# mhvk/baseband

Measured on AMD Instinct MI355X. Metric: decoded Msamples/s, VDIF 2-bit 1-thread (scan + index + decode, input resident in HBM), higher is better.
Workload: dtype float32; 1 GPU; cfg2: synthetic 8.000 GiB per GPU single-thread VDIF, 2-bit real, 1 channel, EDV 0, 8032-byte frames; input_memory=arena, output_memory=torch.empty, 127.5 GiB (above the readers' 64 GiB arena block limit)

## Files before the change

baseband_amd/_lib.py:

```python
import ctypes as C
import os

import torch

_HERE = os.path.dirname(os.path.abspath(__file__))
EXPERIMENTS = os.environ.get('BB_EXPERIMENTS', '') not in ('', '0')
LIB_PATH = os.path.join(_HERE, 'libbbdecode_exp.so' if EXPERIMENTS else 'libbbdecode.so')

BB_OK = 0
BB_EIO = -5
BB_EINVAL = -22
BB_ERANGE = -34
BB_ENOTSUP = -95

CODER_VDIF = 0
CODER_MARK5B = 1
CODER_INT = 2

OUT_F32 = 0
OUT_F16 = 1
OUT_BF16 = 2

FRAME_OK = 0x1
FRAME_INVALID = 0x2
# ... 3 lines not shown
TUNE_ENCODE_DIRECT = 5
TUNE_GATHER_BYTES = 6
TUNE_TILES_PER_WAVE = 7
TUNE_TILED_STAGE = 10
TUNE_MKBF_CHANNELS = 11
TUNE_GATHER_CHUNKS = 12
TUNE_SEG_TILES = 13
TUNE_WORK_STRIPES = 18
TUNE_XPOSE = 19
TUNE_XPOSE_ROWS = 20
TUNE_M4_WIDEN = 22
TUNE_SELECT_BYTES = 23
TUNE_LUT_TILES = 24
TUNE_M4_TILES = 26
TUNE_XPOSE_TC = 27
TUNE_XPOSE_MIN_NC = 28
TUNE_ENCODE_RUNS = 30
TUNE_GATHER_GLDS = 36
TUNE_ENCODE_STRIPES = 38
TUNE_SELECT_PICK = 39
TUNE_PICK_BYTES = 40
TUNE_VDIF8_LDS_GIB = 41
TUNE_TOUCH_MIB = 42
TUNE_FLAT_VARIANT = 0
TUNE_NT_STORES = 1
TUNE_NT_LOADS = 3
TUNE_TILES_PER_WAVE_8BIT = 8
TUNE_LDS_PAD = 9
TUNE_FRONT_GROUP = 14
TUNE_FRONT_STEPS = 15
TUNE_OUT_STRIPE_W = 16
TUNE_OUT_STRIPE_S = 17
TUNE_BYTE_LUT = 21
TUNE_LUT_SMALL = 25
TUNE_FLAT8_LDS = 29
TUNE_BURST = 31
TUNE_COPY = 35
TUNE_M4_LDS = 37
TUNE_BURST_BYTES = 32
TUNE_BURST_PERIOD = 33
TUNE_BURST_WAVES = 34


class BBError(RuntimeError):
    def __init__(self, code, where):
        self.code = code
# ... 162 lines not shown
    ('bb_count_states_bins', C.c_int, [_vp, _sz, _vp, _sz, C.POINTER(StatesParams), C.c_uint64, C.c_uint64,
                                       C.c_uint64, _vp, _sz, _vp]),
    ('bb_count_states_bins_check', C.c_int, [C.POINTER(StatesParams), C.c_uint64]),
    ('bb_i8_moments', C.c_int, [_vp, _sz, _vp, _sz, C.POINTER(MomentsParams), _vp, _sz, _vp]),
    ('bb_i8_moments_check', C.c_int, [C.POINTER(MomentsParams)]),
    ('bb_i8_coherence', C.c_int, [_vp, _sz, _vp, _sz, C.POINTER(MomentsParams), _vp, _sz, _vp]),
    ('bb_i8_coherence_check', C.c_int, [C.POINTER(MomentsParams)]),
    ('bb_repack_frames', C.c_int, [_vp, _sz, _vp, _sz, C.POINTER(RepackParams), _vp, _sz, _vp]),
    ('bb_repack_check', C.c_int, [C.POINTER(RepackParams)]),
    ('bb_requant_frames', C.c_int, [_vp, _sz, _vp, _sz, C.POINTER(RequantParams), _vp, _sz, _vp]),
    ('bb_requant_check', C.c_int, [C.POINTER(RequantParams)]),
    ('bb_recode_frames', C.c_int, [_vp, _sz, _vp, _sz, C.POINTER(RecodeParams), _vp, _sz, _vp]),
    ('bb_recode_check', C.c_int, [C.POINTER(RecodeParams)]),
    ('bb_recode_frames_tables', C.c_int, [_vp, _sz, _vp, _sz, C.POINTER(RecodeParams), _vp, _sz, _vp, _sz, _vp]),
    ('bb_recode_tables_check', C.c_int, [C.POINTER(RecodeParams)]),
    ('bb_fetch_counter', C.c_int, [_vp, _vp, _vp, _vp]),
    ('bb_mark5b_read_window', C.c_int, [_vp, _sz, C.POINTER(Mark5BScanParams), _sz, _sz, C.POINTER(DecodeParams),
                                        _vp, C.c_int, _vp, _vp, _vp, _sz, _sz, _vp, _vp, _vp, _vp]),
    ('bb_mark4_read_window', C.c_int, [_vp, _sz, C.POINTER(Mark4ScanParams), _sz, _sz,
                                       C.POINTER(Mark4DecodeParams), C.c_int, _vp, _vp, _vp, _sz, _sz, _vp, _vp,
                                       _vp, _vp]),
    ('bb_vdif_read_window', C.c_int, [_vp, _sz, C.POINTER(VDIFScanParams), _sz, _vp, _sz, C.POINTER(DecodeParams),
                                      _vp, C.c_int, _vp, _vp, _vp, _sz, C.c_uint32, _sz, _vp, _vp, _vp, _vp]),
    ('bb_mark4_scan', C.c_int, [_vp, _sz, C.POINTER(Mark4ScanParams), _vp, _sz, _vp]),
    ('bb_mark4_locate', C.c_int, [_vp, _sz, C.c_int, _vp, _sz, _vp, _vp]),
    ('bb_mark4_header_crc', C.c_int, [_vp, _sz, C.c_int, _vp, C.c_int64, _sz, _vp, _vp]),
    ('bb_mark4_scan_at', C.c_int, [_vp, _sz, C.POINTER(Mark4ScanParams), _vp, _sz, _vp, _vp]),
    ('bb_decode_mark4', C.c_int, [_vp, _sz, _vp, _sz, C.POINTER(Mark4DecodeParams), _vp, _sz, _vp]),
    ('bb_decode_mark4_select', C.c_int, [_vp, _sz, _vp, _sz, C.POINTER(Mark4DecodeParams), C.c_int,
                                         _vp, _sz, _vp]),
    ('bb_decode_i8_tiled', C.c_int, [_vp, _sz, _vp, _sz, C.POINTER(TiledParams), _vp, _sz, _vp]),
    ('bb_encode_flat', C.c_int, [_vp, _sz, C.c_int, C.c_int, _vp, _sz, _vp]),
    ('bb_encode_mark4', C.c_int, [_vp, _sz, C.c_int, C.POINTER(C.c_uint8), C.POINTER(C.c_uint8), _vp, _sz, _vp]),
    ('bb_tune', C.c_int, [C.c_int, C.c_int]),
    ('bb_arena_create', C.c_int, [_sz, C.POINTER(_vp)]),
    ('bb_arena_alloc', C.c_int, [_vp, _sz, C.POINTER(_vp)]),
    ('bb_arena_prepare', C.c_int, [_vp, _sz]),
    ('bb_arena_owns', C.c_int, [_vp, _vp]),
    ('bb_arena_free', C.c_int, [_vp, _vp]),
    ('bb_arena_trim', C.c_int, [_vp, C.POINTER(_sz)]),
    ('bb_arena_get_stats', C.c_int, [_vp, C.POINTER(ArenaStats)]),
    ('bb_arena_destroy', C.c_int, [_vp]),
]

EXPERIMENT_SIGNATURES = [
    ('bb_debug_trace', C.c_int, [_vp]),
# ... 157 lines not shown
```

baseband_amd/base/base.py:

```python
import operator
import io
import os
import threading
import warnings

import numpy as np
import torch

from .. import _lib
from .. import kernels
from ..placement import empty_output
from .. import placement as _placement
from ..staging import host_image, WindowPipeline
from .packed import PackedBytesMixin
from .quantities import as_time, as_timedelta, is_time_like, is_duration_like

_SIDE_SCAN = os.environ.get('BB_SIDE_SCAN', '1') not in ('0', 'no', 'off')
_scan_streams = {}
_scan_streams_lock = threading.Lock()

__all__ = ['FileBase', 'VLBIFileReaderBase', 'GPUStreamReaderBase',
           'HeaderNotFoundError']


# ... 389 lines not shown
        sub = 'subset={0}, '.format(self.subset) if getattr(self, 'subset', None) else ''
        return ("<{cls} name={name} offset={offset}\n"
                "    sample_rate={rate}, samples_per_frame={spf},\n"
                "    sample_shape={shape}, bps={bps},\n"
                "    {sub}start_time={start}>"
                .format(cls=type(self).__name__, name=getattr(self.fh_raw, 'name', None), offset=attr('offset'),
                        rate=attr('sample_rate'), spf=attr('samples_per_frame'), shape=attr('sample_shape'),
                        bps=attr('bps'), sub=sub, start=attr('start_time')))

    def seekable(self):
        return True

    @property
    def info(self):
        from .info import StreamReaderInfo
        cached = self.__dict__.get('_info')
        if cached is None or cached.verify != self.verify or cached.closed != self.closed:
            cached = self.__dict__['_info'] = StreamReaderInfo(self)
        return cached

    def close(self):
        self._closed = True
        self._drop_windows()
        self._staged = self._sink = None
        self._have = []
        if self._pipeline is not None:
            self._pipeline.release()
            self._pipeline = None
        self.fh_raw.close()
        self._unregister()

    def __enter__(self):
        return self

    def __exit__(self, *exc):
        self.close()

    _within_np = None
    _within_dev = None

    @property
    def _within(self):
        if self._within_np is None:
            return None
        if self._within_dev is None:
            kernels.require_gpu()
# ... 436 lines not shown
                        device=dev, priority=int(os.environ.get('BB_SIDE_SCAN_PRIORITY', '-1')))
            self._scan_stream = st
        key = (resident.data_ptr(), resident.numel(), None if self._nbad is None else self._nbad.data_ptr(),
               self._side_state_key())
        if self._scan_ready_for != key:
            ev = torch.cuda.Event()
            ev.record(torch.cuda.current_stream(dev))
            self._scan_stream.wait_event(ev)
            self._scan_ready_for = key
        return self._scan_stream

    def _side_state_key(self):
        return None

    def _zero_nbad(self):
        if self._nbad is not None:
            if self._scan_stream is not None:
                self._scan_stream.synchronize()
            self._nbad.zero_()
            if self._scan_stream is not None:
                torch.cuda.current_stream(self._nbad.device).synchronize()

    def _reset_checks(self):
        self._nmissing, self._checked, self._check_recs = 0, False, 0
        self._zero_nbad()

    def _fill_request(self, out, count):
        spf = self.samples_per_frame
        first, off0 = divmod(self.offset, spf)
        stop = self.offset + count
        last = -(-stop // spf) if count else first
        flat = self._direct_target(out)
        body0, body1 = first + (1 if off0 else 0), stop // spf
        if flat is not None and count and body1 > body0:
            row = flat.numel() // count
            o0 = body0 * spf - self.offset
            self._read_sets(body0, body1, flat[o0 * row:(o0 + (body1 - body0) * spf) * row])
            if off0:
                head = self._squeeze_and_subset(self._read_sets_as(first, body0, flat.dtype))
                out[:o0] = head[off0:]
            if body1 < last:
                ntail = stop - body1 * spf
                tail = self._squeeze_and_subset(self._read_sets_as(body1, last, flat.dtype))
                out[count - ntail:] = tail[:ntail]
            return out, True
        data = self._read_sets(first, last) if out is None else self._read_sets_as(first, last, self._out_elem(out))
        return data[off0:off0 + count], False
# ... 39 lines not shown
        return flat.reshape(data.shape)

    def _decode_sets(self, first, last, into, elem):
        kernels.require_gpu()
        self._last_scan_side = None
        nsets = last - first
        spf = self.samples_per_frame
        ncomp = 2 if self.complex_data else 1
        row = int(np.prod(self._decode_shape)) * ncomp
        flat = into if into is not None else kernels.empty_decoded(nsets * spf * row, dtype=elem)
        set_nbytes = self._set_nbytes
        resident = self._resident_bytes() if nsets else None
        if resident is None and nsets and self._have:
            lo_ = self._file_offset0 + first * set_nbytes
            hi_ = min(self._file_offset0 + (last + (1 if self.verify else 0)) * set_nbytes,
                      len(self._image()))
            if self._has_bytes(min(lo_, hi_), hi_):
                resident = self._sink[:len(self._image())]
        if resident is not None:
            lo = min(self._file_offset0 + first * set_nbytes, resident.numel())
            look = 1 if self.verify else 0
            hi = max(lo, min(self._file_offset0 + (last + look) * set_nbytes, resident.numel()))
            win = self._device_window(resident, lo, hi)
            if (self.verify and _SIDE_SCAN and nsets * set_nbytes >= (16 << 20)
                    and win.data_ptr() == resident.data_ptr() + lo):
                self._prepare_window_state(win.device)
                self._scan_side = self._scan_stream_for(resident)
            try:
                self._process_window(win, first, last, flat)
            except Exception:
                self._reset_checks()
                raise
            finally:
                self._last_scan_side, self._scan_side = self._scan_side, None
        elif nsets and nsets * set_nbytes * 8 <= self.window_bytes:
            self._read_small(first, last, flat, spf * row)
        elif nsets:
            image = self._image()
            per_win = max(1, self.pipeline_window_bytes // set_nbytes)
            if self._pipeline is None:
                self._pipeline = WindowPipeline(image, (per_win + 1) * set_nbytes)
            sink = self._sink_tensor()
            ranges, spans = [], []
            starts, s = [], first
            for size in ((max(1, per_win // 16), max(1, per_win // 4)) if self.ramp_windows else ()):
                if s < last:
                    starts.append(s)
                    s += size
            starts.extend(range(s, last, per_win))
            for i, s in enumerate(starts):
                e = min(last, starts[i + 1] if i + 1 < len(starts) else s + per_win)
                lo = min(self._file_offset0 + s * set_nbytes, len(image))
                look = 1 if (self.verify and e == last) else 0
                hi = max(lo, min(self._file_offset0 + (e + look) * set_nbytes, len(image)))
                ranges.append((lo, hi))
                spans.append((s, e))

            def process(dbuf, i):
                s, e = spans[i]
                o = flat[(s - first) * spf * row:(e - first) * spf * row]
                self._process_window(self._device_window(dbuf, 0, dbuf.numel()), s, e, o)

            try:
                self._pipeline.run(ranges, process, sink=sink)
            except Exception:
                self._reset_checks()
                raise
            if sink is not None:
                for lo, hi in ranges:
                    self._mark_have(lo, hi)
        if self.complex_data:
            flat = torch.view_as_complex(flat.view(-1, 2))
        return flat.reshape((nsets * spf,) + tuple(self._decode_shape))

    _ahead = None
    _ahead_bytes0 = 256 << 10
    _ahead_bytes = 256 << 10

    def _read_small(self, first, last, flat, set_floats):
        from ..staging import upload
        set_nbytes = self._set_nbytes
        image = self._image()
        total = (len(image) - self._file_offset0) // set_nbytes
        look = 1 if self.verify else 0
        need_end = min(last + look, total)
        ahead = self._ahead
        if ahead is None or first < ahead[0] or need_end > ahead[1]:
            if ahead is not None and ahead[0] <= first <= ahead[1]:
                self._ahead_bytes = min(self.window_bytes, 4 * self._ahead_bytes)
            else:
                self._ahead_bytes = self._ahead_bytes0
            per_win = max(last - first + look, self._ahead_bytes // set_nbytes)
            end = min(total, first + per_win)
            lo = self._file_offset0 + first * set_nbytes
            hi = max(lo, self._file_offset0 + end * set_nbytes)
            dev = upload(image[lo:hi])
# ... 13 lines not shown
    def _note_checked(self, nrecs, missing=0):
        self._check_recs += int(nrecs)
        self._nmissing += int(missing)
        self._checked = True

    def _verdict_targets(self):
        if self._nbad is None:
            self._nbad = torch.zeros(1, dtype=torch.int32, device='cuda')
        if self._check_event is None:
            self._check_event = torch.cuda.Event()
            self._check_event.record()
        return self._nbad, self._check_event.cuda_event

    _check_recs = 0
    _check_event = None
    _check_stream = None
    _nbad_host = None

    def _resolve_checks(self, quiet=False):
        checked, self._checked = self._checked, False
        if not self.verify or not checked:
            return True
        nrecs, self._check_recs = self._check_recs, 0
        if nrecs < 2048:
            nbad = int(self._nbad.item()) + self._nmissing
        else:
            if self._check_stream is None:
                self._check_stream = torch.cuda.Stream(device=self._nbad.device)
                self._nbad_host = torch.zeros(1, dtype=torch.int32, pin_memory=True)
            on_scan = self._last_scan_side
            kernels.fetch_counter(self._nbad, self._nbad_host, None if on_scan is not None else self._check_event,
                                  on_scan if on_scan is not None else self._check_stream)
            nbad = int(self._nbad_host[0]) + self._nmissing
        self._nmissing = 0
        if nbad:
            self._zero_nbad()
            if quiet:
                return False
            msg = ("problem loading frame: {} frame header(s) failed verification "
                   "(bad sync/invariants or unexpected time index)".format(nbad))
            if self.verify == 'fix':
                if self._can_relocate and not self._relocated:
                    return False
                warnings.warn(msg + "; affected samples were set to fill_value.")
            else:
                err = self._verification_error(msg)
                if err is None and self._can_relocate:
                    return False
                raise err if err is not None else ValueError("wrong frame number. " + msg)
        return True

    def _verification_error(self, msg):
        return ValueError("wrong frame number. " + msg)

    _asked = None

# ... 125 lines not shown
```

baseband_amd/csrc/bbdecode.hip:

```cpp
#include "bb_common.h"
#include "k_scan.h"
#include "k_flat.h"
#if BB_EXP
#include "k_exp.h"
#endif
#include "k_lut.h"
#include "k_lds.h"
#include "k_half.h"
#include "bb_half_host.h"
#include "k_copy.h"
#include "k_states.h"
#include "k_state_bins.h"
#include "k_repack.h"
#include "k_requant.h"
#include "k_recode.h"
#include "k_recode_tables.h"
#include "k_moments.h"
#include "k_coherence.h"
#include "k_tfpick.h"
#if BB_EXP
#include "k_burst.h"
#endif
#include "k_gather.h"
#include "k_pick.h"
// ... 141 lines not shown
#define BB_LOCATE_GRID 65536ull

struct bb_knob {
    int v;
    int load() const { return v; }
    bb_knob &operator=(int x) { v = x; return *this; }
};
thread_local bb_knob g_tune_blocks{0};
thread_local bb_knob g_tune_tile_elems{8192};
thread_local bb_knob g_tune_encode_direct{0};
thread_local bb_knob g_tune_gather_bytes{8192};
thread_local bb_knob g_tune_tiled_stage{1};
thread_local bb_knob g_tune_seg_tiles{0};
thread_local bb_knob g_tune_gather_chunks{32};
thread_local bb_knob g_tune_mkbf_tc{32};
thread_local bb_knob g_tune_rows_tiles{8};
thread_local bb_knob g_tune_lut_tpw{0};
static int touch_mib_default()
{
    static const int v = [] { const char *e = getenv("BB_TOUCH_MIB"); char *end = nullptr; const long x = e && *e ? strtol(e, &end, 10) : 256; return (e && *e && end == e) || x < 0 || x > (1 << 20) ? 256 : (int)x; }();
    return v;
}
thread_local bb_knob g_tune_touch_mib{touch_mib_default()};
thread_local bb_knob g_tune_vdif8_lds_gib{20};
thread_local bb_knob g_tune_select_pick{1};
thread_local bb_knob g_tune_pick_bytes{4096};
thread_local bb_knob g_tune_select_bytes{16384};
thread_local bb_knob g_tune_m4_tiles{BB_M4_TPW};
thread_local bb_knob g_tune_m4_widen{1};
thread_local bb_knob g_tune_xpose_rows{0};
#if BB_EXP
thread_local bb_knob g_tune_flat8_lds{0};
#endif
thread_local bb_knob g_tune_encode_runs{0};
thread_local bb_knob g_tune_encode_lw{0};
thread_local bb_knob g_tune_xpose_tc{0};
thread_local bb_knob g_tune_xpose_min_nc{8};
thread_local bb_knob g_tune_xpose{1};
thread_local bb_knob g_tune_gather_glds{-1};
thread_local bb_knob g_tune_order_lw{-1};
#if BB_EXP
thread_local bb_knob g_tune_m4_lds{0};
thread_local bb_knob g_tune_copy{0};
thread_local bb_knob g_tune_variant{5};
thread_local bb_knob g_tune_burst{0};
thread_local bb_knob g_tune_burst_bytes{65536};
// ... 451 lines not shown
    switch (knob) {
        case BB_TUNE_BLOCKS:       g_tune_blocks = value;  return BB_OK;
        case BB_TUNE_TILE_ELEMS:   g_tune_tile_elems = value > 0 ? value : 8192; return BB_OK;
        case BB_TUNE_ENCODE_DIRECT: g_tune_encode_direct = value; return BB_OK;
        case BB_TUNE_TILES_PER_WAVE:
            g_tune_rows_tiles = (value >= 1 && value <= 8) ? value : 8;
#if BB_EXP
            g_tune_tpw = (value >= 1 && value <= 16) ? value : 12;
#endif
            return BB_OK;
        case BB_TUNE_GATHER_BYTES: g_tune_gather_bytes = value > 0 ? value : 8192; return BB_OK;
        case BB_TUNE_TILED_STAGE: g_tune_tiled_stage = value; return BB_OK;
        case BB_TUNE_SEG_TILES: g_tune_seg_tiles = (value >= 1 && value <= 4096) ? value : 0; return BB_OK;
        case BB_TUNE_GATHER_CHUNKS: g_tune_gather_chunks = value > 0 ? value : 32; return BB_OK;
        case BB_TUNE_MKBF_CHANNELS: g_tune_mkbf_tc = (value >= 2 && value <= 64 && !(value & 1)) ? value : 32; return BB_OK;
        case BB_TUNE_M4_WIDEN: g_tune_m4_widen = value; return BB_OK;
        case BB_TUNE_M4_TILES: g_tune_m4_tiles = (value >= 1 && value <= BB_M4_TPW) ? value : BB_M4_TPW; return BB_OK;
        case BB_TUNE_LUT_TILES: g_tune_lut_tpw = (value >= 1 && value <= 16) ? value : 0; return BB_OK;
        case BB_TUNE_SELECT_BYTES:
            if (value < 256 || value > 32768) return BB_EINVAL;
            g_tune_select_bytes = value; return BB_OK;
        case BB_TUNE_VDIF8_LDS_GIB: g_tune_vdif8_lds_gib = value < 0 ? 20 : value; return BB_OK;
        case BB_TUNE_TOUCH_MIB: g_tune_touch_mib = value < 0 ? touch_mib_default() : value; return BB_OK;
        case BB_TUNE_SELECT_PICK: g_tune_select_pick = value < 0 ? 1 : (value > 2 ? 2 : value); return BB_OK;
        case BB_TUNE_PICK_BYTES:
            if (value < 1024 || value > 32768) return BB_EINVAL;
            g_tune_pick_bytes = value; return BB_OK;
        case BB_TUNE_XPOSE: g_tune_xpose = value; return BB_OK;
        case BB_TUNE_XPOSE_ROWS: g_tune_xpose_rows = value == 64 ? 64 : value == 128 ? 128 : 0; return BB_OK;
        case BB_TUNE_ENCODE_RUNS: g_tune_encode_runs = (value == 1 || value == 2) ? value : 0; return BB_OK;
        case BB_TUNE_ENCODE_STRIPES: g_tune_encode_lw = (value >= 0 && value <= 10) ? value : 0; return BB_OK;
        case BB_TUNE_XPOSE_TC: g_tune_xpose_tc = (value == 64 || value == 32 || value == 16 || value == 8) ? value : 0; return BB_OK;
        case BB_TUNE_XPOSE_MIN_NC: g_tune_xpose_min_nc = value < 2 ? 2 : value; return BB_OK;
        case BB_TUNE_GATHER_GLDS: g_tune_gather_glds = value < 0 ? -1 : (value != 0); return BB_OK;
        case BB_TUNE_WORK_STRIPES: g_tune_order_lw = (value >= 0 && value <= 10) ? value : -1; return BB_OK;
#if BB_EXP
        case BB_TUNE_FLAT_VARIANT: g_tune_variant = value; return BB_OK;
        case BB_TUNE_COPY: g_tune_copy = value; return BB_OK;
        case BB_TUNE_M4_LDS: g_tune_m4_lds = value != 0; return BB_OK;
        case BB_TUNE_BURST: g_tune_burst = value; return BB_OK;
        case BB_TUNE_BURST_BYTES: g_tune_burst_bytes = (value >= 4096 && value <= 79360) ? (value & ~255) : 65536; return BB_OK;
        case BB_TUNE_BURST_PERIOD: g_tune_burst_period = value > 0 ? value : 0; return BB_OK;
        case BB_TUNE_BURST_WAVES: g_tune_burst_waves = (value == 3 || value == 7 || value == 15) ? value : 15; return BB_OK;
        case BB_TUNE_FLAT8_LDS: g_tune_flat8_lds = value; return BB_OK;
        case BB_TUNE_NT_STORES:    g_tune_nt = value;      return BB_OK;
        case BB_TUNE_NT_LOADS:     g_tune_nt_loads = value; return BB_OK;
// ... 593 lines not shown
    void *ss;
    int rc = window_begin(d_buf, nbytes, scan && dec, nullptr, 0, verified, scan_stream, stream, &ss);
    if (rc != BB_OK) return rc;
    rc = bb_mark4_scan(d_buf, nbytes, scan, d_recs, nframes, ss);
    if (rc != BB_OK) return rc;
    rc = index_verify(d_recs, nframes, nullptr, 1, d_src, n, false, 1, nstrict, d_nbad, ss);
    if (rc != BB_OK) return rc;
    rc = window_verified(verified, scan_stream, ss, stream);
    if (rc != BB_OK) return rc;
    if (nout > 0)
        return bb_decode_mark4_select(d_buf, nbytes, d_src, n, dec, nout, d_out, out_elems, stream);
    return bb_decode_mark4(d_buf, nbytes, d_src, n, dec, d_out, out_elems, stream);
}

int bb_fetch_counter(const uint32_t *d_counter, uint32_t *h_value, void *after, void *side_stream)
{
    if (!d_counter || !h_value) return BB_EINVAL;
    hipStream_t st = (hipStream_t)side_stream;
    if (after) BB_HIP(hipStreamWaitEvent(st, (hipEvent_t)after, 0));
    BB_HIP(hipMemcpyAsync(h_value, d_counter, sizeof(uint32_t), hipMemcpyDeviceToHost, st));
    BB_HIP(hipStreamSynchronize(st));
    return BB_OK;
}

int bb_copy_frames(const void *d_buf, size_t buf_nbytes, size_t nframes, uint64_t nbytes_per_frame,
                   int64_t src0, int64_t src_stride, void *d_out, size_t out_nbytes, void *stream)
{
    if (nframes == 0 || nbytes_per_frame == 0) { BB_NOTE("none"); return BB_OK; }
    if (!d_buf || !d_out) return BB_EINVAL;
    if ((nbytes_per_frame & 3) || (reinterpret_cast<uintptr_t>(d_buf) & 3) || (reinterpret_cast<uintptr_t>(d_out) & 3))
        return BB_EINVAL;
    if (nframes > 1 && src_stride > 0 && (uint64_t)src_stride < nbytes_per_frame) return BB_EINVAL;
    if ((uint64_t)nframes > (~0ull) / nbytes_per_frame || (uint64_t)nframes * nbytes_per_frame > out_nbytes) return BB_ERANGE;
    int rc = fixed_stride_check(src0, src_stride, 4, nframes, nbytes_per_frame, buf_nbytes);
    if (rc) return rc;
    rc = ensure_init();
    if (rc) return rc;
    bb_copy_args a;
    a.buf = (const uint8_t *)d_buf; a.out = (uint8_t *)d_out;
    a.nframes = nframes; a.n = nbytes_per_frame;
    int nl = 4, ntl = 1;
#if BB_EXP
    { const int cv = g_tune_copy.load(); if (cv) { nl = cv & 0xff; ntl = (cv >> 8) & 1; } }
    if (nl != 2 && nl != 4 && nl != 8 && nl != 16) nl = 4;
#endif
    const uint64_t item = (uint64_t)nl * BB_BLOCK * 16;
// ... 588 lines not shown
```

baseband_amd/kernels.py:

```python
import ctypes as C
import os

import numpy as np
import torch

from . import _lib
from ._lib import lib, check


_gpu_checked = False


def require_gpu():
    global _gpu_checked
    if _gpu_checked:
        return
    if not torch.cuda.is_available():
        raise RuntimeError(
            "baseband_amd needs an MI355X (gfx950) GPU: torch.cuda.is_available() "
            "is False and there is no CPU decode path in this package.")
    _gpu_checked = True


_raw_stream = getattr(torch._C, '_cuda_getCurrentRawStream', None)
# ... 198 lines not shown
        p.coder, p.bps, p.chunk, p.nslot = coder, bps, chunk, nslot
        p.payload_nbytes = payload_nbytes
        p.complex_data = int(bool(complex_data))
        self.set_fill(fill_value)
        self.recs = self.src = self._sets = None

    def run(self, dbuf, ref_frame_nr, nframes, thread_slot, nsets, within, out,
            recs_per_index, nstrict, nbad, verified, scan_stream=None):
        dev = dbuf.device
        self.scan.ref_frame_nr = ref_frame_nr
        if not verified:
            scan_stream = None
        st = self._scratch(nframes, nsets * self.dec.nslot, dev, scan_stream)
        self.dec.out_type = _out_type(out.dtype)
        tgt = _Target(out, out.numel(), dev, out.dtype)
        nsel = within.numel() if within is not None else 0
        check(lib.bb_vdif_read_window(
            _ptr(dbuf), dbuf.numel(), C.byref(self.scan), nframes, _ptr(thread_slot), nsets,
            C.byref(self.dec), _ptr(within), nsel, _ptr(self.recs), _ptr(self.src),
            _ptr(tgt.use), tgt.use.numel(), recs_per_index, nstrict, _ptr(nbad),
            *_side_handles(verified, scan_stream), _stream(dbuf)), 'bb_vdif_read_window')
        self._decode_queued(st, scan_stream, dev)
        tgt.done()


class Mark5BWindow(_FrameWindow):
    __slots__ = ('scan', 'dec')

    def __init__(self, ref_seconds, frame_rate, bps, chunk, fill_value):
        self.scan = _mark5b_params(ref_seconds, 0, frame_rate)
        d = self.dec = _lib.DecodeParams()
        d.coder, d.bps, d.chunk, d.nslot, d.payload_nbytes = _lib.CODER_MARK5B, bps, chunk, 1, 10000
        self.recs = self.src = self._sets = None
        self.set_fill(fill_value)

    def run(self, dbuf, ref_frame_nr, nframes, n, within, out, nstrict, nbad, verified, scan_stream=None):
        self.scan.ref_frame_nr = ref_frame_nr
        if not verified:
            scan_stream = None
        st = self._scratch(nframes, n, dbuf.device, scan_stream)
        self.dec.out_type = _out_type(out.dtype)
        tgt = _Target(out, out.numel(), dbuf.device, out.dtype)
        check(lib.bb_mark5b_read_window(
            _ptr(dbuf), dbuf.numel(), C.byref(self.scan), nframes, n, C.byref(self.dec), _ptr(within),
            within.numel() if within is not None else 0, _ptr(self.recs), _ptr(self.src), _ptr(tgt.use),
            tgt.use.numel(), nstrict, _ptr(nbad), *_side_handles(verified, scan_stream), _stream(dbuf)),
# ... 603 lines not shown
```

baseband_amd/vdif/base.py:

```python

import warnings

import numpy as np
import torch

from .. import _lib, kernels
from ..base.base import (FileBase, VLBIFileReaderBase, GPUStreamReaderBase,
                         HeaderNotFoundError)
from ..base.packed import PackedGeometry
from ..base.writer import GPUStreamWriterBase
from ..base.opener import FormatOpener
from ..base.header import strided_header_words
from .header import VDIFHeader, frame_header_words
from .frame import VDIFFrame, VDIFFrameSet
from ..base.quantities import hz

__all__ = ['VDIFFileReader', 'VDIFFileWriter', 'VDIFStreamReader', 'VDIFStreamWriter',
           'open']


class VDIFFileReader(VLBIFileReaderBase):
    _format = 'vdif'
    _info_find_kwargs = {'maximum': 0}

# ... 512 lines not shown
        nframes = min(nsets * nthread_file, dbuf.numel() // self._frame_nbytes)
        if self._thread_slot is None:
            self._thread_slot = kernels.thread_slot_map(self._thread_ids,
                                                        dbuf.device)
        which = '_window' if self.verify else '_window_unverified'
        w = getattr(self, which)
        if w is None:
            w = kernels.VDIFWindow(
                self._frame_nbytes, h0.nbytes, self._pattern,
                self._mask if self.verify else [0] * len(self._mask), h0['seconds'], self._frame_rate,
                h0.payload_nbytes, self._coder, self.bps, h0.nchan * (2 if self.complex_data else 1),
                len(self._thread_ids), self.complex_data, self.fill_value)
            setattr(self, which, w)
        if w.fill_value != self.fill_value:
            w.set_fill(self.fill_value)
        nbad = verified = None
        if self.verify:
            nbad, verified = self._verdict_targets()
        w.run(dbuf, h0['frame_nr'] + first_set, nframes, self._thread_slot, nsets, self._within, out_flat,
              nthread_file, nframes, nbad, verified, scan_stream=self._scan_side)
        if self.verify:
            self._note_checked(nframes, missing=nsets * nthread_file - nframes)

    def _packed_geometry(self):
        h0 = self.header0
        return PackedGeometry(self._coder, self.bps, h0.nchan * (2 if self.complex_data else 1),
                              len(self._thread_ids), h0.payload_nbytes)

    def _packed_index(self, dbuf, first, nsets, verdict=None):
        h0 = self.header0
        nslot = len(self._thread_ids)
        nthread_file = len(self._file_threads)
        nframes = min(nsets * nthread_file, dbuf.numel() // self._frame_nbytes)
        if verdict is not None:
            verdict.missing += nsets * nthread_file - nframes
        if nframes == 0:
            return torch.full((nsets * nslot,), -1, dtype=torch.int64, device=dbuf.device)
        if self._thread_slot is None:
            self._thread_slot = kernels.thread_slot_map(self._thread_ids, dbuf.device)
        recs = kernels.vdif_scan(dbuf, nframes, self._frame_nbytes, h0.nbytes, self._pattern,
                                 self._mask if self.verify else [0] * len(self._mask), h0['seconds'],
                                 h0['frame_nr'] + first, self._frame_rate, set_nframes=nthread_file)
        if verdict is not None:
            kernels.verify_records(recs, nframes, 0, nthread_file, nframes, verdict.counter)
        return kernels.build_index(recs, nsets, nslot, self._thread_slot)

# ... 134 lines not shown
```

include/bbdecode.h:

```cpp
#ifndef BBDECODE_H
#define BBDECODE_H

#include <stddef.h>
#include <stdint.h>

#ifdef __cplusplus
extern "C" {
#endif

#define BB_ABI_VERSION 7

#define BB_OK        0
#define BB_EIO      (-5)
#define BB_EINVAL   (-22)
#define BB_ERANGE   (-34)
#define BB_ENOTSUP  (-95)

enum bb_coder {
    BB_CODER_VDIF   = 0,
    BB_CODER_MARK5B = 1,
    BB_CODER_INT    = 2
};

enum bb_out_type {
// ... 109 lines not shown
                            float *d_out, size_t out_elems, void *stream);

int bb_decode_frames_select_check(const bb_decode_params *params, int nwithin);

int bb_vdif_read_window(const void *d_buf, size_t nbytes,
                        const bb_vdif_scan_params *scan, size_t nframes,
                        const int16_t *d_thread_slot, size_t nsets,
                        const bb_decode_params *dec,
                        const int32_t *d_within, int nwithin,
                        bb_frame_rec *d_recs, int64_t *d_src,
                        float *d_out, size_t out_elems,
                        uint32_t recs_per_index, size_t nstrict, uint32_t *d_nbad,
                        void *verified, void *scan_stream, void *stream);

int bb_mark5b_read_window(const void *d_buf, size_t nbytes,
                          const bb_mark5b_scan_params *scan, size_t nframes, size_t n,
                          const bb_decode_params *dec,
                          const int32_t *d_within, int nwithin,
                          bb_frame_rec *d_recs, int64_t *d_src,
                          float *d_out, size_t out_elems,
                          size_t nstrict, uint32_t *d_nbad, void *verified, void *scan_stream, void *stream);

int bb_fetch_counter(const uint32_t *d_counter, uint32_t *h_value, void *after, void *side_stream);


typedef struct bb_mark4_scan_params {
    uint64_t first_offset;
    int32_t  ntrack;
    int32_t  ref_year;
    int64_t  ref_qms;
    int32_t  frame_qms;
    int32_t  by_position;
} bb_mark4_scan_params;

int bb_mark4_scan(const void *d_buf, size_t nbytes,
                  const bb_mark4_scan_params *params,
                  bb_frame_rec *d_recs, size_t nframes, void *stream);

int bb_mark4_header_crc(const void *d_buf, size_t nbytes, int ntrack,
                        const int64_t *d_offsets, int64_t first_offset, size_t nframes,
                        uint64_t *d_bad_tracks, void *stream);

int bb_mark4_locate(const void *d_buf, size_t nbytes, int ntrack,
                    int64_t *d_offsets, size_t cap,
                    unsigned long long *d_count, void *stream);
int bb_mark4_scan_at(const void *d_buf, size_t nbytes,
// ... 206 lines not shown
```

include/bbdecode_tune.h:

```cpp
#ifndef BBDECODE_TUNE_H
#define BBDECODE_TUNE_H

#ifdef __cplusplus
extern "C" {
#endif

#define BB_TUNE_BLOCKS         2
#define BB_TUNE_TILE_ELEMS     4
#define BB_TUNE_ENCODE_DIRECT  5
#define BB_TUNE_GATHER_BYTES   6
#define BB_TUNE_TILES_PER_WAVE 7
#define BB_TUNE_TILED_STAGE   10
#define BB_TUNE_MKBF_CHANNELS 11
#define BB_TUNE_GATHER_CHUNKS 12
#define BB_TUNE_SEG_TILES     13
#define BB_TUNE_WORK_STRIPES  18
#define BB_TUNE_XPOSE         19
#define BB_TUNE_XPOSE_ROWS    20
#define BB_TUNE_M4_WIDEN      22
#define BB_TUNE_SELECT_BYTES  23
#define BB_TUNE_LUT_TILES     24
#define BB_TUNE_XPOSE_TC      27
#define BB_TUNE_XPOSE_MIN_NC  28
#define BB_TUNE_ENCODE_RUNS   30
#define BB_TUNE_M4_TILES      26
#define BB_TUNE_GATHER_GLDS   36
#define BB_TUNE_SELECT_PICK    39
#define BB_TUNE_PICK_BYTES     40
#define BB_TUNE_VDIF8_LDS_GIB   41
#define BB_TUNE_TOUCH_MIB       42
#define BB_TUNE_ENCODE_STRIPES 38

int bb_tune(int knob, int value);

#ifdef __cplusplus
}
#endif
#endif
```

Baseline: 1.621 million Msamples/s.

## Add persistent native VDIF reader handle for HBM-resident window reads

Adds a persistent C-side VDIF reader object that owns scratch record/index buffers, a side scan stream and events, and performs scan, index-verify and decode in one native call per window. The Python read path tries this native reader first when the window is in place, falling back to the existing window-processing path otherwise. The aim is to cut per-read Python, ctypes and allocation overhead and keep buffers reused across reads. In exchange, the verify path does a blocking host sync for the bad-frame count on every read, and the extra handle state adds complexity.

```diff
diff --git a/baseband_amd/_lib.py b/baseband_amd/_lib.py
--- a/baseband_amd/_lib.py
+++ b/baseband_amd/_lib.py
@@ -49,6 +49,7 @@
 TUNE_PICK_BYTES = 40
 TUNE_VDIF8_LDS_GIB = 41
 TUNE_TOUCH_MIB = 42
+TUNE_NATIVE_READ = 43
 TUNE_FLAT_VARIANT = 0
 TUNE_NT_STORES = 1
 TUNE_NT_LOADS = 3
@@ -257,6 +258,13 @@
                                        _vp, _vp]),
     ('bb_vdif_read_window', C.c_int, [_vp, _sz, C.POINTER(VDIFScanParams), _sz, _vp, _sz, C.POINTER(DecodeParams),
                                       _vp, C.c_int, _vp, _vp, _vp, _sz, C.c_uint32, _sz, _vp, _vp, _vp, _vp]),
+    ('bb_vdif_reader_create', C.c_int, [C.POINTER(VDIFScanParams), C.POINTER(DecodeParams), _vp, C.c_int, _vp, C.c_int,
+                                        C.c_int, C.POINTER(_vp)]),
+    ('bb_vdif_reader_destroy', C.c_int, [_vp]),
+    ('bb_vdif_reader_set_fill', C.c_int, [_vp, C.c_float, C.c_float]),
+    ('bb_vdif_reader_read', C.c_int, [_vp, _vp, _sz, C.c_int32, _sz, _sz, _sz, _vp, _sz, C.c_int, C.c_int, _vp,
+                                      C.POINTER(C.c_uint32)]),
+    ('bb_native_read', C.c_int, []),
     ('bb_mark4_scan', C.c_int, [_vp, _sz, C.POINTER(Mark4ScanParams), _vp, _sz, _vp]),
     ('bb_mark4_locate', C.c_int, [_vp, _sz, C.c_int, _vp, _sz, _vp, _vp]),
     ('bb_mark4_header_crc', C.c_int, [_vp, _sz, C.c_int, _vp, C.c_int64, _sz, _vp, _vp]),
diff --git a/baseband_amd/base/base.py b/baseband_amd/base/base.py
--- a/baseband_amd/base/base.py
+++ b/baseband_amd/base/base.py
@@ -435,6 +435,7 @@
     def close(self):
         self._closed = True
         self._drop_windows()
+        self._drop_native()
         self._staged = self._sink = None
         self._have = []
         if self._pipeline is not None:
@@ -917,7 +918,7 @@
                 torch.cuda.current_stream(self._nbad.device).synchronize()
 
     def _reset_checks(self):
-        self._nmissing, self._checked, self._check_recs = 0, False, 0
+        self._nmissing, self._checked, self._check_recs, self._native_nbad = 0, False, 0, None
         self._zero_nbad()
 
     def _fill_request(self, out, count):
@@ -1003,17 +1004,10 @@
             look = 1 if self.verify else 0
             hi = max(lo, min(self._file_offset0 + (last + look) * set_nbytes, resident.numel()))
             win = self._device_window(resident, lo, hi)
-            if (self.verify and _SIDE_SCAN and nsets * set_nbytes >= (16 << 20)
-                    and win.data_ptr() == resident.data_ptr() + lo):
-                self._prepare_window_state(win.device)
-                self._scan_side = self._scan_stream_for(resident)
-            try:
-                self._process_window(win, first, last, flat)
-            except Exception:
-                self._reset_checks()
-                raise
-            finally:
-                self._last_scan_side, self._scan_side = self._scan_side, None
+            in_place = win.data_ptr() == resident.data_ptr() + lo
+            if not (_SIDE_SCAN and in_place and kernels.native_read()
+                    and self._read_native(win, resident, first, last, flat)):
+                self._read_window_in_hbm(win, resident, in_place, first, last, flat)
         elif nsets and nsets * set_nbytes * 8 <= self.window_bytes:
             self._read_small(first, last, flat, spf * row)
         elif nsets:
@@ -1053,6 +1047,29 @@
         if self.complex_data:
             flat = torch.view_as_complex(flat.view(-1, 2))
         return flat.reshape((nsets * spf,) + tuple(self._decode_shape))
+
+    def _read_window_in_hbm(self, win, resident, in_place, first, last, flat):
+        if self.verify and _SIDE_SCAN and (last - first) * self._set_nbytes >= (16 << 20) and in_place:
+            self._prepare_window_state(win.device)
+            self._scan_side = self._scan_stream_for(resident)
+        try:
+            self._process_window(win, first, last, flat)
+        except Exception:
+            self._reset_checks()
+            raise
+        finally:
+            self._last_scan_side, self._scan_side = self._scan_side, None
+
+    def _read_native(self, win, resident, first, last, flat):
+        return False
+
+    _native_nbad = None
+    _native = None
+
+    def _drop_native(self):
+        handles, self._native = self._native, None
+        for _, handle in (handles or {}).values():
+            handle.close()
 
     _ahead = None
     _ahead_bytes0 = 256 << 10
@@ -1112,8 +1129,11 @@
         if not self.verify or not checked:
             return True
         nrecs, self._check_recs = self._check_recs, 0
-        if nrecs < 2048:
-            nbad = int(self._nbad.item()) + self._nmissing
+        native, self._native_nbad = self._native_nbad, None
+        if native is not None and not nrecs:
+            nbad = native + self._nmissing
+        elif nrecs < 2048:
+            nbad = int(self._nbad.item()) + self._nmissing + (native or 0)
         else:
             if self._check_stream is None:
                 self._check_stream = torch.cuda.Stream(device=self._nbad.device)
@@ -1121,7 +1141,7 @@
             on_scan = self._last_scan_side
             kernels.fetch_counter(self._nbad, self._nbad_host, None if on_scan is not None else self._check_event,
                                   on_scan if on_scan is not None else self._check_stream)
-            nbad = int(self._nbad_host[0]) + self._nmissing
+            nbad = int(self._nbad_host[0]) + self._nmissing + (native or 0)
         self._nmissing = 0
         if nbad:
             self._zero_nbad()
diff --git a/baseband_amd/csrc/bb_reader.inc b/baseband_amd/csrc/bb_reader.inc
--- /dev/null
+++ b/baseband_amd/csrc/bb_reader.inc
@@ -0,0 +1,209 @@
+
+#define BB_READER_NSETS 4
+#define BB_READER_SIDE_RECS 2048
+
+struct bb_vdif_reader {
+    bb_vdif_scan_params scan;
+    bb_decode_params dec;
+    const int16_t *d_thread_slot;
+    const int32_t *d_within;
+    int nthread_file, nwithin, device;
+    hipStream_t side;
+    hipEvent_t verified;
+    hipEvent_t ready;
+    void *last_stream;
+    bool met;
+    struct {
+        bb_frame_rec *recs;
+        int64_t *src;
+        hipEvent_t decoded;
+        void *by;
+        bool used;
+    } sets[BB_READER_NSETS];
+    void *scratch;
+    size_t cap_recs, cap_src;
+    unsigned turn;
+    uint32_t *d_nbad, *h_nbad;
+};
+
+static int side_priority()
+{
+    const char *e = getenv("BB_SIDE_SCAN_PRIORITY");
+    char *end = nullptr;
+    const long x = e && *e ? strtol(e, &end, 10) : -1;
+    return (e && *e && end == e) ? -1 : (x < 0 ? -1 : 0);
+}
+
+static size_t reader_pow2(size_t n)
+{
+    size_t c = 64;
+    while (c < n) c <<= 1;
+    return c;
+}
+
+static int reader_grow(bb_vdif_reader *h, size_t nrecs, size_t nsrc)
+{
+    for (auto &s : h->sets)
+        if (s.used) { BB_HIP(hipEventSynchronize(s.decoded)); s.used = false; }
+    BB_HIP(hipStreamSynchronize(h->side));
+    int prev = 0;
+    BB_HIP(hipGetDevice(&prev));
+    if (prev != h->device) BB_HIP(hipSetDevice(h->device));
+    const size_t cr = reader_pow2(nrecs > h->cap_recs ? nrecs : h->cap_recs);
+    const size_t cs = reader_pow2(nsrc > h->cap_src ? nsrc : h->cap_src);
+    hipError_t e = hipSuccess;
+    if (h->scratch) e = hipFree(h->scratch);
+    h->scratch = nullptr;
+    h->cap_recs = h->cap_src = 0;
+    if (e == hipSuccess)
+        e = hipMalloc(&h->scratch, BB_READER_NSETS * (cr * sizeof(bb_frame_rec) + cs * sizeof(int64_t)));
+    if (prev != h->device) (void)hipSetDevice(prev);
+    BB_HIP(e);
+    bb_frame_rec *recs = (bb_frame_rec *)h->scratch;
+    int64_t *src = (int64_t *)(recs + BB_READER_NSETS * cr);
+    for (int k = 0; k < BB_READER_NSETS; ++k) {
+        h->sets[k].recs = recs + (size_t)k * cr;
+        h->sets[k].src = src + (size_t)k * cs;
+    }
+    h->cap_recs = cr;
+    h->cap_src = cs;
+    return BB_OK;
+}
+
+static int reader_init(bb_vdif_reader *h)
+{
+    int least = 0, greatest = 0;
+    BB_HIP(hipDeviceGetStreamPriorityRange(&least, &greatest));
+    BB_HIP(hipStreamCreateWithPriority(&h->side, hipStreamNonBlocking, side_priority() < 0 ? greatest : 0));
+    BB_HIP(hipEventCreateWithFlags(&h->verified, hipEventDisableTiming));
+    BB_HIP(hipEventCreateWithFlags(&h->ready, hipEventDisableTiming));
+    for (auto &s : h->sets) BB_HIP(hipEventCreateWithFlags(&s.decoded, hipEventDisableTiming));
+    BB_HIP(hipMalloc((void **)&h->d_nbad, sizeof(uint32_t)));
+    BB_HIP(hipHostMalloc((void **)&h->h_nbad, sizeof(uint32_t), hipHostMallocDefault));
+    *h->h_nbad = 0;
+    BB_HIP(hipMemsetAsync(h->d_nbad, 0, sizeof(uint32_t), h->side));
+    if (int rc = reader_grow(h, 4096, 4096 * (size_t)h->dec.nslot)) return rc;
+    BB_HIP(hipStreamSynchronize(h->side));
+    return BB_OK;
+}
+
+int bb_vdif_reader_destroy(bb_vdif_reader *h)
+{
+    if (!h) return BB_OK;
+    for (auto &s : h->sets)
+        if (s.used) (void)hipEventSynchronize(s.decoded);
+    if (h->side) (void)hipStreamSynchronize(h->side);
+    if (h->scratch) (void)hipFree(h->scratch);
+    if (h->d_nbad) (void)hipFree(h->d_nbad);
+    if (h->h_nbad) (void)hipHostFree(h->h_nbad);
+    for (auto &s : h->sets)
+        if (s.decoded) (void)hipEventDestroy(s.decoded);
+    if (h->ready) (void)hipEventDestroy(h->ready);
+    if (h->verified) (void)hipEventDestroy(h->verified);
+    if (h->side) (void)hipStreamDestroy(h->side);
+    delete h;
+    return BB_OK;
+}
+
+int bb_vdif_reader_create(const bb_vdif_scan_params *scan, const bb_decode_params *dec,
+                          const int16_t *d_thread_slot, int nthread_file,
+                          const int32_t *d_within, int nwithin, int device, bb_vdif_reader **out)
+{
+    if (out) *out = nullptr;
+    if (!scan || !dec || !d_thread_slot || !out) return BB_EINVAL;
+    if (nthread_file < 1 || dec->nslot < 1 || device < 0) return BB_EINVAL;
+    if (nwithin < 0 || (nwithin > 0) != (d_within != nullptr)) return BB_EINVAL;
+    int ndev = 0, prev = 0;
+    if (hipGetDeviceCount(&ndev) != hipSuccess || device >= ndev) return BB_EINVAL;
+    BB_HIP(hipGetDevice(&prev));
+    if (prev != device) BB_HIP(hipSetDevice(device));
+    bb_vdif_reader *h = new bb_vdif_reader();
+    h->scan = *scan;
+    h->scan.set_nframes = nthread_file;
+    h->dec = *dec;
+    h->d_thread_slot = d_thread_slot;
+    h->d_within = d_within;
+    h->nthread_file = nthread_file;
+    h->nwithin = nwithin;
+    h->device = device;
+    int rc = ensure_init();
+    if (rc == BB_OK) rc = reader_init(h);
+    if (prev != device) (void)hipSetDevice(prev);
+    if (rc != BB_OK) { bb_vdif_reader_destroy(h); return rc; }
+    *out = h;
+    return BB_OK;
+}
+
+int bb_vdif_reader_set_fill(bb_vdif_reader *h, float fill_re, float fill_im)
+{
+    if (!h) return BB_EINVAL;
+    h->dec.fill_re = fill_re;
+    h->dec.fill_im = fill_im;
+    return BB_OK;
+}
+
+static int reader_abandon(bb_vdif_reader *h, void *ss, int verify, int rc)
+{
+    if (verify) {
+        (void)hipStreamSynchronize((hipStream_t)ss);
+        (void)hipMemsetAsync(h->d_nbad, 0, sizeof(uint32_t), (hipStream_t)ss);
+        (void)hipStreamSynchronize((hipStream_t)ss);
+    }
+    return rc;
+}
+
+int bb_vdif_reader_read(bb_vdif_reader *h, const void *d_buf, size_t nbytes, int32_t ref_frame_nr,
+                        size_t nframes, size_t nsets, size_t nstrict, void *d_out, size_t out_elems,
+                        int out_type, int verify, void *stream, uint32_t *nbad)
+{
+    if (!h || (verify && !nbad)) return BB_EINVAL;
+    if (nbad) *nbad = 0;
+    bb_decode_params dec = h->dec;
+    dec.out_type = out_type;
+    int rc = window_out_check(&dec, h->nwithin);
+    if (rc != BB_OK) return rc;
+    const size_t nsrc = nsets * (size_t)dec.nslot;
+    const bool aside = verify && nframes >= BB_READER_SIDE_RECS;
+    void *ss = aside ? (void *)h->side : stream;
+    if (aside && (!h->met || stream != h->last_stream)) {
+        BB_HIP(hipEventRecord(h->ready, (hipStream_t)stream));
+        BB_HIP(hipStreamWaitEvent(h->side, h->ready, 0));
+        h->met = true;
+        h->last_stream = stream;
+    }
+    rc = touch_window(d_buf, nbytes, stream);
+    if (rc != BB_OK) return rc;
+    if (nframes > h->cap_recs || nsrc > h->cap_src) {
+        rc = reader_grow(h, nframes, nsrc);
+        if (rc != BB_OK) return rc;
+    }
+    auto &set = h->sets[h->turn++ % BB_READER_NSETS];
+    if (set.used && set.by != ss) BB_HIP(hipStreamWaitEvent((hipStream_t)ss, set.decoded, 0));
+    bb_vdif_scan_params sp = h->scan;
+    sp.ref_frame_nr = ref_frame_nr;
+    rc = vdif_scan_impl(d_buf, nbytes, &sp, set.recs, nframes, set.src, nsrc, ss);
+    if (rc != BB_OK) return rc;
+    rc = index_verify(set.recs, nframes, h->d_thread_slot, dec.nslot, set.src, nsets, true,
+                      (uint32_t)h->nthread_file, nstrict, verify ? h->d_nbad : nullptr, ss);
+    if (rc != BB_OK) return reader_abandon(h, ss, verify, rc);
+    if (aside) {
+        rc = window_verified(h->verified, h->side, ss, stream);
+        if (rc != BB_OK) return reader_abandon(h, ss, verify, rc);
+    }
+    rc = h->nwithin > 0
+        ? bb_decode_frames_select(d_buf, nbytes, set.src, nsets, &dec, h->d_within, h->nwithin,
+                                  (float *)d_out, out_elems, stream)
+        : bb_decode_frames(d_buf, nbytes, set.src, nsets, &dec, (float *)d_out, out_elems, stream);
+    if (rc != BB_OK) return reader_abandon(h, ss, verify, rc);
+    if (hipEventRecord(set.decoded, (hipStream_t)stream) != hipSuccess)
+        return reader_abandon(h, ss, verify, hip_fail(hipGetLastError()));
+    set.used = true;
+    set.by = stream;
+    if (verify) {
+        BB_HIP(hipMemcpyAsync(h->h_nbad, h->d_nbad, sizeof(uint32_t), hipMemcpyDeviceToHost, (hipStream_t)ss));
+        BB_HIP(hipStreamSynchronize((hipStream_t)ss));
+        *nbad = *h->h_nbad;
+        if (*nbad) return reader_abandon(h, ss, 1, BB_OK);
+    }
+    return BB_OK;
+}
diff --git a/baseband_amd/csrc/bbdecode.hip b/baseband_amd/csrc/bbdecode.hip
--- a/baseband_amd/csrc/bbdecode.hip
+++ b/baseband_amd/csrc/bbdecode.hip
@@ -187,6 +187,12 @@
     return v;
 }
 thread_local bb_knob g_tune_touch_mib{touch_mib_default()};
+static int native_read_default()
+{
+    static const int v = [] { const char *e = getenv("BB_NATIVE_READ"); char *end = nullptr; const long x = e && *e ? strtol(e, &end, 10) : 1; return (e && *e && end == e) ? 1 : (x != 0); }();
+    return v;
+}
+thread_local bb_knob g_tune_native_read{native_read_default()};
 thread_local bb_knob g_tune_vdif8_lds_gib{20};
 thread_local bb_knob g_tune_select_pick{1};
 thread_local bb_knob g_tune_pick_bytes{4096};
@@ -684,6 +690,7 @@
             g_tune_select_bytes = value; return BB_OK;
         case BB_TUNE_VDIF8_LDS_GIB: g_tune_vdif8_lds_gib = value < 0 ? 20 : value; return BB_OK;
         case BB_TUNE_TOUCH_MIB: g_tune_touch_mib = value < 0 ? touch_mib_default() : value; return BB_OK;
+        case BB_TUNE_NATIVE_READ: g_tune_native_read = value < 0 ? native_read_default() : (value != 0); return BB_OK;
         case BB_TUNE_SELECT_PICK: g_tune_select_pick = value < 0 ? 1 : (value > 2 ? 2 : value); return BB_OK;
         case BB_TUNE_PICK_BYTES:
             if (value < 1024 || value > 32768) return BB_EINVAL;
@@ -1323,6 +1330,10 @@
     BB_HIP(hipStreamSynchronize(st));
     return BB_OK;
 }
+
+#include "bb_reader.inc"
+
+int bb_native_read(void) { return g_tune_native_read.load(); }
 
 int bb_copy_frames(const void *d_buf, size_t buf_nbytes, size_t nframes, uint64_t nbytes_per_frame,
                    int64_t src0, int64_t src_stride, void *d_out, size_t out_nbytes, void *stream)
diff --git a/baseband_amd/kernels.py b/baseband_amd/kernels.py
--- a/baseband_amd/kernels.py
+++ b/baseband_amd/kernels.py
@@ -244,6 +244,58 @@
             *_side_handles(verified, scan_stream), _stream(dbuf)), 'bb_vdif_read_window')
         self._decode_queued(st, scan_stream, dev)
         tgt.done()
+
+
+def native_read():
+    return lib.bb_native_read() != 0
+
+
+class VDIFReader:
+    __slots__ = ('handle', 'fill_value', '_keep', '_nbad', '_nbad_ref', '_read')
+
+    def __init__(self, frame_nbytes, header_nbytes, pattern, mask, ref_seconds, frame_rate,
+                 payload_nbytes, coder, bps, chunk, nslot, complex_data, fill_value,
+                 thread_slot, nthread_file, within):
+        scan = _vdif_params(frame_nbytes, header_nbytes, pattern, mask, ref_seconds, 0, frame_rate)
+        p = _lib.DecodeParams()
+        p.coder, p.bps, p.chunk, p.nslot = coder, bps, chunk, nslot
+        p.payload_nbytes = payload_nbytes
+        p.complex_data = int(bool(complex_data))
+        fv = complex(fill_value)
+        p.fill_re, p.fill_im = fv.real, fv.imag
+        self.fill_value = fill_value
+        self._keep = (thread_slot, within)
+        self._nbad = C.c_uint32(0)
+        self._nbad_ref = C.byref(self._nbad)
+        self._read = lib.bb_vdif_reader_read
+        self.handle = None
+        h = C.c_void_p(0)
+        check(lib.bb_vdif_reader_create(C.byref(scan), C.byref(p), _ptr(thread_slot), nthread_file, _ptr(within),
+                                        within.numel() if within is not None else 0,
+                                        thread_slot.device.index, C.byref(h)), 'bb_vdif_reader_create')
+        self.handle = h
+
+    def set_fill(self, fill_value):
+        fv = complex(fill_value)
+        check(lib.bb_vdif_reader_set_fill(self.handle, fv.real, fv.imag), 'bb_vdif_reader_set_fill')
+        self.fill_value = fill_value
+
+    def read(self, dbuf, ref_frame_nr, nframes, nsets, nstrict, out, verify):
+        check(self._read(self.handle, dbuf.data_ptr(), dbuf.numel(), ref_frame_nr, nframes, nsets, nstrict,
+                         out.data_ptr(), out.numel(), _out_type(out.dtype), 1 if verify else 0,
+                         _stream(dbuf), self._nbad_ref), 'bb_vdif_reader_read')
+        return self._nbad.value
+
+    def close(self):
+        h, self.handle = self.handle, None
+        if h is not None:
+            lib.bb_vdif_reader_destroy(h)
+
+    def __del__(self):
+        try:
+            self.close()
+        except Exception:
+            pass
 
 
 class Mark5BWindow(_FrameWindow):
diff --git a/baseband_amd/vdif/base.py b/baseband_amd/vdif/base.py
--- a/baseband_amd/vdif/base.py
+++ b/baseband_amd/vdif/base.py
@@ -558,6 +558,46 @@
         if self.verify:
             self._note_checked(nframes, missing=nsets * nthread_file - nframes)
 
+    def _read_native(self, win, resident, first, last, flat):
+        nsets = last - first
+        nthread_file = len(self._file_threads)
+        nframes = min(nsets * nthread_file, win.numel() // self._frame_nbytes)
+        within = self._within
+        if (not nframes or flat.data_ptr() % 16 or not flat.is_contiguous()
+                or (within is not None and flat.dtype != torch.float32)):
+            return False
+        if self._thread_slot is None:
+            self._thread_slot = kernels.thread_slot_map(self._thread_ids, win.device)
+        verify = bool(self.verify)
+        key = (resident.data_ptr(), resident.numel(), self._thread_slot.data_ptr(),
+               None if within is None else within.data_ptr())
+        made = self._native.get(verify) if self._native else None
+        if made is None or made[0] != key:
+            if made is not None:
+                made[1].close()
+            h0 = self.header0
+            made = (key, kernels.VDIFReader(
+                self._frame_nbytes, h0.nbytes, self._pattern,
+                self._mask if verify else [0] * len(self._mask), h0['seconds'], self._frame_rate,
+                h0.payload_nbytes, self._coder, self.bps, h0.nchan * (2 if self.complex_data else 1),
+                len(self._thread_ids), self.complex_data, self.fill_value,
+                self._thread_slot, nthread_file, within))
+            if self._native is None:
+                self._native = {}
+            self._native[verify] = made
+        reader = made[1]
+        if reader.fill_value != self.fill_value:
+            reader.set_fill(self.fill_value)
+        try:
+            nbad = reader.read(win, self.header0['frame_nr'] + first, nframes, nsets, nframes, flat, verify)
+        except Exception:
+            self._reset_checks()
+            raise
+        if verify:
+            self._native_nbad = (self._native_nbad or 0) + nbad
+            self._note_checked(0, missing=nsets * nthread_file - nframes)
+        return True
+
     def _packed_geometry(self):
         h0 = self.header0
         return PackedGeometry(self._coder, self.bps, h0.nchan * (2 if self.complex_data else 1),
diff --git a/include/bbdecode.h b/include/bbdecode.h
--- a/include/bbdecode.h
+++ b/include/bbdecode.h
@@ -155,6 +155,16 @@
                           size_t nstrict, uint32_t *d_nbad, void *verified, void *scan_stream, void *stream);
 
 int bb_fetch_counter(const uint32_t *d_counter, uint32_t *h_value, void *after, void *side_stream);
+
+typedef struct bb_vdif_reader bb_vdif_reader;
+int bb_vdif_reader_create(const bb_vdif_scan_params *scan, const bb_decode_params *dec,
+                          const int16_t *d_thread_slot, int nthread_file,
+                          const int32_t *d_within, int nwithin, int device, bb_vdif_reader **out);
+int bb_vdif_reader_destroy(bb_vdif_reader *h);
+int bb_vdif_reader_set_fill(bb_vdif_reader *h, float fill_re, float fill_im);
+int bb_vdif_reader_read(bb_vdif_reader *h, const void *d_buf, size_t nbytes, int32_t ref_frame_nr,
+                        size_t nframes, size_t nsets, size_t nstrict, void *d_out, size_t out_elems,
+                        int out_type, int verify, void *stream, uint32_t *nbad);
 
 
 typedef struct bb_mark4_scan_params {
diff --git a/include/bbdecode_tune.h b/include/bbdecode_tune.h
--- a/include/bbdecode_tune.h
+++ b/include/bbdecode_tune.h
@@ -29,9 +29,12 @@
 #define BB_TUNE_PICK_BYTES     40
 #define BB_TUNE_VDIF8_LDS_GIB   41
 #define BB_TUNE_TOUCH_MIB       42
+#define BB_TUNE_NATIVE_READ     43
 #define BB_TUNE_ENCODE_STRIPES 38
 
 int bb_tune(int knob, int value);
+
+int bb_native_read(void);
 
 #ifdef __cplusplus
 }
```

Result: no change. 1.619 million Msamples/s (-0.1%).
